# sarvex/redpanda

Hardware: AMD Instinct MI355X
Metric: record-batch validate+parse(+decompress) GB/s per GPU and per 8-GPU node (higher is better)
Workload: dtype u8; 1 GPU; C2: 1,048,576 uncompressed Kafka v2 batches x 16,381 B (16 records x (16 B key + 995 B value)), 4096 partitions per GPU; Kafka CRC32C + internal header CRC + record walk + offset/timestamp index; batches_per_gpu=1048576, batches_total=1048576, partitions_total=4096, partitions_per_gpu=4096, parallelism=partition-shard x1

## Files before the change

redpanda_amd/csrc/rpgpu_kernels.hip:

```cpp
#include "rpgpu_device.h"
#include "rpgpu_walk.h"

namespace rpgpu {

#ifdef RPGPU_DIAG_STAMPS
__device__ unsigned long long g_stamps[8];
struct Stamps {
    uint64_t st[8];
    uint64_t prev;
};
#define DIAG_PARAM , Stamps& sp
#define DIAG_PASS , sp
#define STAMP(i)                                          \
    do {                                                  \
        const uint64_t _t = __builtin_amdgcn_s_memtime(); \
        sp.st[i] += _t - sp.prev;                         \
        sp.prev = _t;                                     \
    } while (0)
#else
#define DIAG_PARAM
#define DIAG_PASS
#define STAMP(i) \
    do {         \
    } while (0)
#endif

struct Header {
    int32_t size_bytes;
    int64_t base_offset;
    int32_t type;
    int32_t crc;
    int16_t attrs;
    int32_t last_offset_delta;
    int64_t first_ts, max_ts, producer_id;
    int16_t producer_epoch;
    int32_t base_sequence, record_count;
};

struct Result {
    int32_t verdict;
    uint32_t crc, crc_expected, header_crc;
    Header h;
    uint32_t index_first, index_count;
};

__device__ __forceinline__ uint32_t u32s(uint32_t v) { return (uint32_t)__builtin_amdgcn_readfirstlane((int)v); }
__device__ __forceinline__ void write_result(rpgpu_batch_result* out, const Result& r) {
    if (lane_id() == 0) {
        const uint64_t bo = (uint64_t)r.h.base_offset, ft = (uint64_t)r.h.first_ts, mt = (uint64_t)r.h.max_ts;
        u32x4 a = {u32s((uint32_t)r.verdict), u32s(r.crc), u32s(r.crc_expected), u32s(r.header_crc)};
        u32x4 b = {u32s((uint32_t)r.h.size_bytes), u32s((uint32_t)r.h.record_count), u32s((uint32_t)bo),
                   u32s((uint32_t)(bo >> 32))};
        u32x4 c = {u32s((uint32_t)r.h.last_offset_delta),
                   u32s((uint32_t)(uint16_t)r.h.attrs | ((uint32_t)(r.h.attrs & 7) << 16) |
                        ((uint32_t)(uint8_t)r.h.type << 24)),
                   u32s((uint32_t)ft), u32s((uint32_t)(ft >> 32))};
        u32x4 d = {u32s((uint32_t)mt), u32s((uint32_t)(mt >> 32)), u32s(r.index_first), u32s(r.index_count)};
        u32x4* o = reinterpret_cast<u32x4*>(out);
        o[0] = a;
        o[1] = b;
        o[2] = c;
        o[3] = d;
    }
}

__device__ __forceinline__ void load_tables(uint32_t* s, const uint32_t* __restrict__ g) {
    for (int i = threadIdx.x; i < kTableWords / 4; i += blockDim.x)
        reinterpret_cast<u32x4*>(s)[i] = reinterpret_cast<const u32x4*>(g)[i];
    __syncthreads();
}

__device__ __forceinline__ uint32_t header_crc_vec(const uint32_t* sT, const Img64& D) {
    uint32_t win[16];
    win[0] = 0;
    win[1] = (D.w[1] << 24) ^ 0xff000000u;
    win[2] = ((D.w[1] >> 8) | (D.w[2] << 24)) ^ 0x00ffffffu;
#pragma unroll
    for (int m = 3; m < 16; m++) win[m] = (D.w[m - 1] >> 8) | (D.w[m] << 24);
    const uint32_t l = lane_id();
    uint32_t vwin = 0;
#pragma unroll
    for (int i = 0; i < 16; i++) vwin = writelane(vwin, win[i], i);
    const uint32_t w = __builtin_amdgcn_ds_bpermute((int)((l >> 2) << 2), vwin);
    const uint32_t byte = (w >> (8 * (l & 3))) & 255u;
    const uint32_t* hb = sT + kOffHB + l;
    uint32_t c = hb[(byte & 15u) * 64] ^ hb[(16u + (byte >> 4)) * 64];
    c ^= row_shl<1>(c);
    c ^= row_shl<2>(c);
    c ^= row_shl<4>(c);
    c ^= row_shl<8>(c);
    return ~(rdl(c, 0) ^ rdl(c, 16) ^ rdl(c, 32) ^ rdl(c, 48));
}

struct Geom {
    int32_t niter, g0;
};
__device__ __forceinline__ Geom geometry(int32_t n) {
    const int32_t niter = (n - 21 + 1023) >> 10;
    return Geom{niter, n - (niter << 10)};
}
__device__ __forceinline__ int32_t chunk_rows(int32_t niter) {
    return (niter + kRowsPerChunk - 1) & ~(kRowsPerChunk - 1);
}

struct Prefetch {
    u32x4 x[kRowsPerChunk];
    uint32_t hv;
    Geom gm;
};

typedef int32_t i32x4 __attribute__((ext_vector_type(4)));
__device__ __forceinline__ __amdgpu_buffer_rsrc_t batch_rsrc(const uint8_t* p) {
    return __builtin_amdgcn_make_buffer_rsrc(const_cast<uint8_t*>(p), 0, 0x7ffffff0, 0x00020000);
}
#ifndef RPGPU_ROW_AUX
#define RPGPU_ROW_AUX 2
#endif
__device__ __forceinline__ u32x4 load_row(__amdgpu_buffer_rsrc_t rs, const Geom& gm, int32_t row, uint32_t l) {
    const int32_t rb = row < gm.niter ? gm.g0 + (row << 10) : (int32_t)0x80000000;
    const i32x4 v = __builtin_amdgcn_raw_buffer_load_b128(rs, rb + (int32_t)(16 * l), 0, RPGPU_ROW_AUX);
    return (u32x4){(uint32_t)v.x, (uint32_t)v.y, (uint32_t)v.z, (uint32_t)v.w};
}

__device__ __forceinline__ void load_rows(u32x4 (&x)[kRowsPerChunk], __amdgpu_buffer_rsrc_t rs, const Geom& gm,
                                          int32_t cb, uint32_t l) {
#pragma unroll
    for (int k = 0; k < kRowsPerChunk; k++) x[k] = load_row(rs, gm, cb + k, l);
}

__device__ __forceinline__ Geom desc_geometry(const rpgpu_batch_desc& d) {
    return (d.length >= (uint32_t)kHeaderSize && !(d.flags & RPGPU_DESC_NULL_RECORDS)) ? geometry((int32_t)d.length)
                                                                                      : Geom{0, 0};
}

__device__ __forceinline__ u32x4 merge_header(u32x4 y, int32_t ro0, uint32_t v_img, uint32_t l) {
    if (ro0 >= kHeaderSize) return y;
    const int32_t ro = ro0 + 16 * (int32_t)l;
#pragma unroll
    for (int q = 0; q < 4; q++) {
        const int32_t o4 = ro + 4 * q;
        const uint32_t im = img_dword(v_img, o4);
        uint32_t keep;
        if (o4 >= kHeaderSize)
            keep = 0xffffffffu;
        else if (o4 + 4 <= kHeaderSize)
            keep = 0;
        else
            keep = 0xffffffffu << (8 * (uint32_t)(kHeaderSize - o4));
        const uint32_t raw = q == 0 ? y.x : q == 1 ? y.y : q == 2 ? y.z : y.w;
        const uint32_t v = (raw & keep) | (o4 >= kHeaderSize ? 0u : im);
        if (q == 0) y.x = v;
        if (q == 1) y.y = v;
        if (q == 2) y.z = v;
        if (q == 3) y.w = v;
    }
    return y;
}

__device__ __forceinline__ void process_batch(const uint32_t* __restrict__ sT, const rpgpu_batch_desc& d,
                                              uint32_t b, const uint8_t* __restrict__ data,
                                              rpgpu_batch_result* __restrict__ res, uint32_t index_first,
                                              Prefetch& pf, const rpgpu_batch_desc& nd,
                                              bool has_next DIAG_PARAM) {
    const uint32_t l = lane_id();
    const uint8_t* p = data + d.offset;
    const uint32_t len = d.length;
    Result r;
    r.verdict = RPGPU_V_OK;
    r.crc = r.crc_expected = r.header_crc = 0;
    r.h.size_bytes = r.h.type = r.h.crc = r.h.last_offset_delta = 0;
    r.h.base_sequence = r.h.record_count = 0;
    r.h.attrs = r.h.producer_epoch = 0;
    r.h.base_offset = r.h.first_ts = r.h.max_ts = r.h.producer_id = 0;
    r.index_first = index_first;
    r.index_count = 0;

    const uint32_t hv = pf.hv;
    Img64 H;
#pragma unroll
    for (int i = 0; i < 16; i++) H.w[i] = rdl(hv, i);
    Geom ngm{0, 0};
    const __amdgpu_buffer_rsrc_t nrs = batch_rsrc(data + (has_next ? nd.offset : 0));
    pf.hv = (uint32_t)__builtin_amdgcn_raw_buffer_load_b32(nrs, (int32_t)(4 * (l & 15)), 0, 0);
    if (has_next) ngm = desc_geometry(nd);

    Img64 D;
    D.clear();
    int64_t n;
    bool body_trunc = false;
    bool fail = false;
    if (d.flags & RPGPU_DESC_NULL_RECORDS) {
        n = 0;
        r.verdict = RPGPU_V_NULL_RECORDS;
        fail = true;
    } else if (d.format == RPGPU_FMT_KAFKA_WIRE) {
        const int32_t bl = (int32_t)H.get_be(8, 4);
        const uint64_t blen = (uint64_t)(int64_t)bl + 12u;
        if (blen <= (uint64_t)len) {
            n = (int64_t)blen;
        } else {
            n = len;
            body_trunc = true;
        }
        if (len < 12) {
            r.verdict = RPGPU_V_TOO_SMALL;
            fail = true;
        } else if (n < 17) {
            r.verdict = RPGPU_V_HDR_TRUNC_THROW;
            fail = true;
        } else if ((int8_t)H.byte(16) != 2) {
            r.verdict = RPGPU_V_BAD_MAGIC;
            fail = true;
        } else if (n < kHeaderSize) {
            r.verdict = RPGPU_V_HDR_TRUNC_THROW;
            fail = true;
        } else {
            r.h.size_bytes = (int32_t)((uint32_t)bl + 12u);
            r.h.base_offset = (int64_t)H.get_be(0, 8);
            r.h.type = 1;
            r.h.crc = (int32_t)H.get_be(17, 4);
            r.h.attrs = (int16_t)H.get_be(21, 2);
            r.h.last_offset_delta = (int32_t)H.get_be(23, 4);
            r.h.first_ts = (int64_t)H.get_be(27, 8);
            r.h.max_ts = (int64_t)H.get_be(35, 8);
            r.h.producer_id = (int64_t)H.get_be(43, 8);
            r.h.producer_epoch = (int16_t)H.get_be(51, 2);
            r.h.base_sequence = (int32_t)H.get_be(53, 4);
            r.h.record_count = (int32_t)H.get_be(57, 4);
            D.put_le(4, (uint32_t)r.h.size_bytes, 4);
            D.put_le(8, (uint64_t)r.h.base_offset, 8);
            D.put_le(16, 1, 1);
            D.put_le(17, (uint32_t)r.h.crc, 4);
            D.put_le(21, (uint16_t)r.h.attrs, 2);
            D.put_le(23, (uint32_t)r.h.last_offset_delta, 4);
            D.put_le(27, (uint64_t)r.h.first_ts, 8);
            D.put_le(35, (uint64_t)r.h.max_ts, 8);
            D.put_le(43, (uint64_t)r.h.producer_id, 8);
            D.put_le(51, (uint16_t)r.h.producer_epoch, 2);
            D.put_le(53, (uint32_t)r.h.base_sequence, 4);
            D.put_le(57, (uint32_t)r.h.record_count, 4);
        }
    } else {
        n = 0;
        if (len < kHeaderSize) {
            r.verdict = RPGPU_V_STREAM_SHORT;
            fail = true;
        } else {
            uint32_t any = 0;
#pragma unroll
            for (int i = 0; i < 15; i++) any |= H.w[i];
            any |= H.w[15] & 0xffu;
            if (any == 0) {
                r.verdict = RPGPU_V_FALLOCATED_ZERO;
                fail = true;
            } else {
#pragma unroll
                for (int i = 0; i < 16; i++) D.w[i] = H.w[i];
                D.w[15] &= 0xffu;
                r.h.size_bytes = (int32_t)H.get_le(4, 4);
                r.h.base_offset = (int64_t)H.get_le(8, 8);
                r.h.type = (int8_t)H.byte(16);
                r.h.crc = (int32_t)H.get_le(17, 4);
                r.h.attrs = (int16_t)H.get_le(21, 2);
                r.h.last_offset_delta = (int32_t)H.get_le(23, 4);
                r.h.first_ts = (int64_t)H.get_le(27, 8);
                r.h.max_ts = (int64_t)H.get_le(35, 8);
                r.h.producer_id = (int64_t)H.get_le(43, 8);
                r.h.producer_epoch = (int16_t)H.get_le(51, 2);
                r.h.base_sequence = (int32_t)H.get_le(53, 4);
                r.h.record_count = (int32_t)H.get_le(57, 4);
                n = (int64_t)r.h.size_bytes;
            }
        }
    }
    const bool is_disk = d.format != RPGPU_FMT_KAFKA_WIRE;
    const bool recrc = is_disk && (d.ops & RPGPU_OP_RECRC);
    if (!fail) {
        r.crc_expected = (uint32_t)r.h.crc;
        if (!recrc && ((d.ops & RPGPU_OP_HDRCRC) || is_disk)) r.header_crc = header_crc_vec(sT, D);
        if (is_disk) {
            if (!recrc && r.header_crc != H.w[0]) {
                r.verdict = RPGPU_V_HDR_CRC_MISMATCH;
                fail = true;
            } else if (r.h.size_bytes < kHeaderSize || (int64_t)r.h.size_bytes > (int64_t)len) {
                r.verdict = RPGPU_V_STREAM_SHORT;
                fail = true;
            }
        }
    }
    if (fail) {
        load_rows(pf.x, nrs, ngm, 0, l);
        pf.gm = ngm;
        write_result(res + b, r);
        return;
    }

    Img64 B;
    B.clear();
    B.put_be(21, (uint16_t)r.h.attrs, 2);
    B.put_be(23, (uint32_t)r.h.last_offset_delta, 4);
    B.put_be(27, (uint64_t)r.h.first_ts, 8);
    B.put_be(35, (uint64_t)r.h.max_ts, 8);
    B.put_be(43, (uint64_t)r.h.producer_id, 8);
    B.put_be(51, (uint16_t)r.h.producer_epoch, 2);
    B.put_be(53, (uint32_t)r.h.base_sequence, 4);
    B.put_be(57, (uint32_t)r.h.record_count, 4);
    B.w[5] ^= 0xffffff00u;
    B.w[6] ^= 0x000000ffu;
    uint32_t v_img = 0;
#pragma unroll
    for (int i = 0; i < 16; i++) v_img = (l == (uint32_t)i) ? B.w[i] : v_img;

    const Geom gm = geometry((int32_t)n);
    const int32_t nrows = chunk_rows(gm.niter);
    const bool pf_ok = pf.gm.niter == gm.niter && pf.gm.g0 == gm.g0;
    const uint32_t* sN = sT + kOffN;
    const __amdgpu_buffer_rsrc_t rs = batch_rsrc(p);
    const __amdgpu_buffer_rsrc_t nrs_rows = batch_rsrc(data + (has_next ? nd.offset : 0));
    uint32_t c = 0;
    STAMP(0);
    if (!pf_ok) load_rows(pf.x, rs, gm, 0, l);
    pf.x[0] = merge_header(pf.x[0], gm.g0, v_img, l);
    pf.x[1] = merge_header(pf.x[1], gm.g0 + 1024, v_img, l);
    for (int32_t cb = 0; cb < nrows; cb += kRowsPerChunk) {
        const bool last_chunk = cb + kRowsPerChunk >= nrows;
        const __amdgpu_buffer_rsrc_t lrs = last_chunk ? nrs_rows : rs;
        const Geom lg = last_chunk ? ngm : gm;
        const int32_t lrow = last_chunk ? 0 : cb + kRowsPerChunk;
#pragma unroll
        for (int k = 0; k < kRowsPerChunk; k++) {
            u32x4 y = pf.x[k];
            y.x ^= c;
            c = crc_block(sN, y);
            pf.x[k] = load_row(lrs, lg, lrow + k, l);
        }
    }
    pf.gm = ngm;
    STAMP(1);
#ifndef RPGPU_DIAG_NO_COMBINE
    c = combine64(sT + kOffW, c);
    if (nrows != gm.niter) c = apply8(sT + kOffU + (nrows - gm.niter) * 128, c);
#endif
    r.crc = ~rdl(c, 0);
#if defined(RPGPU_DIAG_NO_COMBINE) || defined(RPGPU_DIAG_NO_LOOKUP)
    asm volatile("" ::"v"(c));
    r.crc = r.crc_expected;
#endif
    if (recrc) {
        r.crc_expected = r.crc;
        r.h.crc = (int32_t)r.crc;
        D.put_le(17, r.crc, 4);
        r.header_crc = header_crc_vec(sT, D);
    }
    STAMP(2);

    const uint8_t codec = (uint8_t)(r.h.attrs & 7);
    if (r.crc != r.crc_expected) {
        r.verdict = RPGPU_V_CRC_MISMATCH;
    } else if (body_trunc) {
        r.verdict = RPGPU_V_BODY_TRUNC_THROW;
    } else if (codec > 4) {
        r.verdict = RPGPU_V_BAD_CODEC_THROW;
    }
    write_result(res + b, r);
    STAMP(3);
}

__global__ __launch_bounds__(kValidateThreads) void validate_kernel(
    const rpgpu_batch_desc* __restrict__ descs, uint32_t b0, uint32_t n, const uint8_t* __restrict__ data,
    rpgpu_batch_result* __restrict__ res, rpgpu_record_index* __restrict__ index,
    const uint32_t* __restrict__ local_first, const uint32_t* __restrict__ caps,
    const uint64_t* __restrict__ block_base, uint64_t index_cap, const uint32_t* __restrict__ tables) {
    __shared__ __attribute__((aligned(16))) uint32_t sT[kTableWords];
    load_tables(sT, tables);
    const uint32_t wave = threadIdx.x >> 6;
    const uint32_t gw = __builtin_amdgcn_readfirstlane(blockIdx.x * kWavesPerBlock + wave);
    const uint32_t nw = gridDim.x * kWavesPerBlock;
#ifdef RPGPU_DIAG_STAMPS
    Stamps sp{};
    sp.prev = __builtin_amdgcn_s_memtime();
#endif
    Prefetch pf;
    pf.gm = Geom{0, 0};
    if (b0 + gw < n) {
        const rpgpu_batch_desc d0 = sload_desc(descs + b0 + gw);
        const uint8_t* p0 = data + d0.offset;
        const __amdgpu_buffer_rsrc_t rs0 = batch_rsrc(p0);
        pf.hv = (uint32_t)__builtin_amdgcn_raw_buffer_load_b32(rs0, (int32_t)(4 * (lane_id() & 15)), 0, 0);
        pf.gm = desc_geometry(d0);
        load_rows(pf.x, rs0, pf.gm, 0, lane_id());
    }
    for (uint32_t b = b0 + gw; b < n; b += nw) {
        const rpgpu_batch_desc d = sload_desc(descs + b);
        const bool has_next = b + nw < n;
        const rpgpu_batch_desc nd = sload_desc(descs + (has_next ? b + nw : b));
        process_batch(sT, d, b, data, res, 0u, pf, nd, has_next DIAG_PASS);
        STAMP(5);
    }
#ifdef RPGPU_DIAG_STAMPS
    if (lane_id() == 0)
        for (int i = 0; i < 6; i++) atomicAdd(&g_stamps[i], (unsigned long long)sp.st[i]);
#endif
}

__global__ __launch_bounds__(256) void walk_kernel(const rpgpu_batch_desc* __restrict__ descs, uint32_t b0,
                                                   uint32_t n,
                                                   const uint8_t* __restrict__ data,
                                                   rpgpu_batch_result* __restrict__ res,
                                                   rpgpu_record_index* __restrict__ index,
                                                   const uint32_t* __restrict__ local_first,
                                                   const uint32_t* __restrict__ caps,
                                                   const uint64_t* __restrict__ block_base, uint64_t index_cap,
                                                   uint32_t* __restrict__ wave_list, uint32_t* __restrict__ wave_count) {
    const uint32_t b = b0 + blockIdx.x * blockDim.x + threadIdx.x;
    WalkJob J;
    J.flags = 0;
    J.body = 0;
    J.base_offset = J.first_ts = 0;
    J.n = J.first = J.cap = J.b = 0;
    J.rc = 0;
    uint32_t first_all = 0;
    if (b < n) {
        const rpgpu_batch_desc d = descs[b];
        const rpgpu_batch_result& r = res[b];
        const uint64_t first = block_base[b / kScanBlock] + local_first[b];
        first_all = (uint32_t)first;
        if ((d.ops & (RPGPU_OP_PARSE | RPGPU_OP_INDEX)) && r.verdict == RPGPU_V_OK && r.codec == 0) {
            uint64_t cap = caps[b];
            if (first >= index_cap) cap = 0;
            else if (first + cap > index_cap) cap = index_cap - first;
            J.body = d.offset + kHeaderSize;
            J.base_offset = r.base_offset;
            J.first_ts = r.first_timestamp;
            J.n = (uint32_t)r.size_bytes - kHeaderSize;
            J.rc = r.record_count;
            J.first = (uint32_t)first;
            J.cap = (uint32_t)cap;
            J.b = b;
            J.flags = kJobLive | ((d.ops & RPGPU_OP_INDEX) ? kJobIndex : 0u);
            if (J.rc > kWaveWalkMin) {
                wave_list[atomicAdd(wave_count, 1u)] = b;
                J.flags = 0;
            }
        }
    }
    walk_lanes(data, J, index, res);
    if (b < n && !(J.flags & kJobLive)) reinterpret_cast<uint32_t*>(res + b)[14] = first_all;
}

__global__ __launch_bounds__(256) void walk_wave_kernel(const rpgpu_batch_desc* __restrict__ descs,
                                                        const uint8_t* __restrict__ data,
                                                        rpgpu_batch_result* __restrict__ res,
                                                        rpgpu_record_index* __restrict__ index,
                                                        const uint32_t* __restrict__ local_first,
                                                        const uint32_t* __restrict__ caps,
                                                        const uint64_t* __restrict__ block_base, uint64_t index_cap,
                                                        const uint32_t* __restrict__ wave_list,
                                                        const uint32_t* __restrict__ wave_count,
                                                        uint32_t* __restrict__ head) {
    const uint32_t cnt = *wave_count;
    for (;;) {
        uint32_t k = 0;
        if (lane_id() == 0) k = atomicAdd(head, 1u);
        k = __builtin_amdgcn_readfirstlane(k);
        if (k >= cnt) break;
        const uint32_t b = wave_list[k];
        const rpgpu_batch_desc d = descs[b];
        const rpgpu_batch_result& r = res[b];
        const uint64_t first = block_base[b / kScanBlock] + local_first[b];
        uint64_t cap = caps[b];
        if (first >= index_cap) cap = 0;
        else if (first + cap > index_cap) cap = index_cap - first;
        WalkJob J;
        J.body = d.offset + kHeaderSize;
        J.base_offset = r.base_offset;
        J.first_ts = r.first_timestamp;
        J.n = (uint32_t)r.size_bytes - kHeaderSize;
        J.rc = r.record_count;
        J.first = (uint32_t)first;
        J.cap = (uint32_t)cap;
        J.b = b;
        J.flags = kJobLive | ((d.ops & RPGPU_OP_INDEX) ? kJobIndex : 0u);
        int32_t verdict;
        uint32_t count;
        wave_walk_batch(data, J, index, verdict, count);
        if (lane_id() == 0) {
            uint32_t* o = reinterpret_cast<uint32_t*>(res + b);
            o[0] = (uint32_t)verdict;
            o[15] = count;
        }
    }
}

__device__ __forceinline__ uint32_t index_cap(const rpgpu_batch_desc& d, const uint8_t* data) {
    if (!(d.ops & (RPGPU_OP_PARSE | RPGPU_OP_INDEX)) || (d.flags & RPGPU_DESC_NULL_RECORDS)) return 0;
    const uint8_t* p = data + d.offset;
    const uint64_t len = d.length;
    if (len < (uint64_t)kHeaderSize) return 0;
    uint64_t n;
    int32_t rc;
    uint32_t attrs;
    if (d.format == RPGPU_FMT_KAFKA_WIRE) {
        const int32_t bl = (int32_t)bswap32(ld4(p + 8));
        const uint64_t blen = (uint64_t)(int64_t)bl + 12u;
        if (blen > len) return 0;
        n = blen;
        if (n < (uint64_t)kHeaderSize || p[16] != 2) return 0;
        attrs = ((uint32_t)p[21] << 8) | p[22];
        rc = (int32_t)bswap32(ld4(p + 57));
    } else {
        const int32_t sz = (int32_t)ld4(p + 4);
        if (sz < kHeaderSize || (uint64_t)sz > len) return 0;
        n = (uint64_t)sz;
        attrs = ((uint32_t)p[22] << 8) | p[21];
        rc = (int32_t)ld4(p + 57);
    }
    if ((attrs & 7u) != 0 || rc <= 0) return 0;
    uint64_t cap = (n - kHeaderSize) / 2;
    if ((uint64_t)rc < cap) cap = (uint64_t)rc;
    return (uint32_t)cap;
}

__global__ __launch_bounds__(kScanBlock) void caps_kernel(const rpgpu_batch_desc* __restrict__ descs,
                                                          uint32_t n, const uint8_t* __restrict__ data,
                                                          uint32_t* __restrict__ caps,
                                                          uint32_t* __restrict__ local_first,
                                                          uint64_t* __restrict__ block_sum) {
    __shared__ uint32_t wsum[kScanBlock / 64];
    const uint32_t i = blockIdx.x * kScanBlock + threadIdx.x;
    uint32_t cap = 0;
    if (i < n) cap = index_cap(descs[i], data);
    const uint32_t l = lane_id();
    uint32_t x = cap;
#pragma unroll
    for (int s = 1; s < 64; s <<= 1) {
        uint32_t t = __shfl_up(x, s, 64);
        if (l >= (uint32_t)s) x += t;
    }
    const uint32_t wv = threadIdx.x >> 6;
    if (l == 63) wsum[wv] = x;
    __syncthreads();
    uint32_t wbase = 0;
    for (uint32_t k = 0; k < wv; k++) wbase += wsum[k];
    if (i < n) {
        caps[i] = cap;
        local_first[i] = wbase + x - cap;
    }
    if (threadIdx.x == kScanBlock - 1) {
        uint64_t tot = 0;
        for (uint32_t k = 0; k < kScanBlock / 64; k++) tot += wsum[k];
        block_sum[blockIdx.x] = tot;
    }
}

__global__ __launch_bounds__(1024) void block_scan_kernel(uint64_t* __restrict__ block_sum, uint32_t nb,
                                                          uint64_t* __restrict__ total_out) {
    __shared__ uint64_t part[1024];
    const uint32_t t = threadIdx.x;
    const uint32_t per = (nb + 1023) / 1024;
    const uint32_t lo = t * per, hi = (lo + per < nb) ? lo + per : nb;
    uint64_t s = 0;
    for (uint32_t k = lo; k < hi; k++) s += block_sum[k];
    part[t] = s;
    __syncthreads();
    for (uint32_t off = 1; off < 1024; off <<= 1) {
        uint64_t v = (t >= off) ? part[t - off] : 0;
        __syncthreads();
        part[t] += v;
        __syncthreads();
    }
    uint64_t run = part[t] - s;
    for (uint32_t k = lo; k < hi; k++) {
        const uint64_t v = block_sum[k];
        block_sum[k] = run;
        run += v;
    }
    if (t == 1023 && total_out) *total_out = part[1023];
}

__global__ __launch_bounds__(kValidateThreads) void crc_ranges_kernel(
    const uint8_t* __restrict__ data, const uint64_t* __restrict__ offs, const uint32_t* __restrict__ lens,
    const uint32_t* __restrict__ seeds, uint32_t n, uint32_t* __restrict__ out,
    const uint32_t* __restrict__ tables) {
    __shared__ __attribute__((aligned(16))) uint32_t sT[kTableWords];
    load_tables(sT, tables);
    const uint32_t l = lane_id();
    const uint32_t wave = threadIdx.x >> 6;
    const uint32_t gw = __builtin_amdgcn_readfirstlane(blockIdx.x * kWavesPerBlock + wave);
    const uint32_t nw = gridDim.x * kWavesPerBlock;
    for (uint32_t i = gw; i < n; i += nw) {
        const uint8_t* base = data + offs[i];
        const int64_t len = lens[i];
        const uint32_t init = ~(seeds ? seeds[i] : 0u);
        const uint32_t crc = crc_range_wave(sT, base, len, init, l);
        if (l == 0) out[i] = crc;
    }
}

__device__ __forceinline__ bool header_all_zero(const Img64& H) {
    uint32_t any = 0;
#pragma unroll
    for (int i = 0; i < 15; i++) any |= H.w[i];
    any |= H.w[15] & 0xffu;
    return any == 0;
}

__global__ __launch_bounds__(kValidateThreads) void segment_parse_kernel(
    const uint8_t* __restrict__ data, const rpgpu_segment_read* __restrict__ reads, uint32_t nreads,
    rpgpu_segment_parse_result* __restrict__ results, rpgpu_batch_desc* __restrict__ descs,
    const uint32_t* __restrict__ tables) {
    __shared__ __attribute__((aligned(16))) uint32_t sT[kTableWords];
    load_tables(sT, tables);
    const uint32_t l = lane_id();
    const uint32_t gw = __builtin_amdgcn_readfirstlane(blockIdx.x * kWavesPerBlock + (threadIdx.x >> 6));
    const uint32_t nw = gridDim.x * kWavesPerBlock;
    for (uint32_t s = gw; s < nreads; s += nw) {
        const rpgpu_segment_read rd = reads[s];
        const uint8_t* seg = data + rd.offset;
        const uint64_t len = rd.length;
        const bool reader = rd.mode == RPGPU_PARSE_READER;
        const uint64_t max_buffer = rd.max_buffer ? rd.max_buffer : 32u * 1024u;
        uint64_t pos = 0, bytes_consumed = 0, phys = 0, buffer = 0;
        int32_t err = RPGPU_V_OK;
        bool exception = false, stopped = false, over_budget = false;
        bool codec_throw = false;
        uint32_t accepted = 0, skipped = 0;
        int64_t start_offset = rd.start_offset, expected = rd.expected_next_batch;
        uint64_t cfg_bytes = rd.bytes_consumed;
        const __amdgpu_buffer_rsrc_t rs = batch_rsrc(seg);
        for (;;) {
            const uint64_t rem = len - pos;
            if (rem == 0) {
                err = RPGPU_V_END_OF_STREAM;
                break;
            }
            if (rem < (uint64_t)kHeaderSize) {
                err = RPGPU_V_STREAM_SHORT;
                break;
            }
            const uint32_t hv = (uint32_t)__builtin_amdgcn_raw_buffer_load_b32(rs, (int32_t)(pos + 4 * (l & 15)), 0, 0);
            Img64 H;
#pragma unroll
            for (int i = 0; i < 16; i++) H.w[i] = rdl(hv, i);
            if (header_all_zero(H)) {
                err = RPGPU_V_FALLOCATED_ZERO;
                break;
            }
            Img64 D;
#pragma unroll
            for (int i = 0; i < 16; i++) D.w[i] = H.w[i];
            D.w[15] &= 0xffu;
            if (header_crc_vec(sT, D) != H.w[0]) {
                err = RPGPU_V_HDR_CRC_MISMATCH;
                break;
            }
            const int32_t size_bytes = (int32_t)H.get_le(4, 4);
            const int64_t base_offset = (int64_t)H.get_le(8, 8);
            const int8_t type = (int8_t)H.byte(16);
            const int32_t lod = (int32_t)H.get_le(23, 4);
            const int64_t max_ts = (int64_t)H.get_le(35, 8);
            const int64_t last = base_offset + lod;
            const uint64_t sz = (uint64_t)(int64_t)size_bytes;
            int decision = 0;
            if (reader) {
                if (base_offset < expected) {
                    exception = true;
                    break;
                }
                if (base_offset > rd.max_offset) {
                    decision = 2;
                } else if ((rd.strict_max_bytes || cfg_bytes) && cfg_bytes + sz > rd.max_bytes) {
                    over_budget = true;
                    decision = 2;
                } else if (last < start_offset) {
                    decision = 1;
                } else if (rd.has_type_filter && rd.type_filter != type) {
                    start_offset = last + 1;
                    decision = 1;
                } else if (rd.has_first_timestamp && rd.first_timestamp > max_ts) {
                    start_offset = last + 1;
                    decision = 1;
                }
            }
            if (decision == 2) {
                stopped = true;
                break;
            }
            const uint64_t body = (uint64_t)((int64_t)size_bytes - kHeaderSize);
            const uint64_t avail = len - pos - kHeaderSize;
            if (decision == 1) {
                expected = last + 1;
                phys += sz;
                if (body > avail) {
                    err = RPGPU_V_STREAM_SHORT;
                    break;
                }
                pos += kHeaderSize + body;
                bytes_consumed += sz;
                skipped++;
                continue;
            }
            if (reader) expected = last + 1;
            phys += sz;
            const bool throws = reader && (H.byte(21) & 7u) > 4u && body <= avail;
            if (!throws && accepted < rd.desc_cap && l == 0) {
                rpgpu_batch_desc d;
                d.offset = rd.offset + pos;
                d.length = (uint32_t)(body > avail ? avail + kHeaderSize : body + kHeaderSize);
                d.partition = rd.partition;
                d.format = RPGPU_FMT_RP_DISK;
                d.ops = rd.ops;
                d.flags = 0;
                d.reserved = 0;
                descs[rd.desc_first + accepted] = d;
            }
            if (!throws) accepted++;
            bytes_consumed += sz;
            if (body > avail) {
                err = RPGPU_V_STREAM_SHORT;
                break;
            }
            pos += kHeaderSize + body;
            if (throws) {
                codec_throw = true;
                break;
            }
            if (reader) {
                start_offset = last + 1;
                cfg_bytes += sz;
                buffer += sz;
                if (last >= rd.stable_offset || last >= rd.max_offset ||
                    (rd.has_next_cached && rd.next_cached_batch == last + 1) || cfg_bytes >= rd.max_bytes ||
                    buffer >= max_buffer) {
                    stopped = true;
                    break;
                }
            }
        }
        if (l == 0) {
            rpgpu_segment_parse_result r;
            r.last_error = (exception || codec_throw) ? RPGPU_V_OK : err;
            const bool benign = err == RPGPU_V_OK || err == RPGPU_V_END_OF_STREAM || err == RPGPU_V_FALLOCATED_ZERO;
            r.status = exception     ? RPGPU_V_READ_OFFSET_REGRESSION
                       : codec_throw ? RPGPU_V_BAD_CODEC_THROW
                                     : ((bytes_consumed || benign) ? RPGPU_V_OK : err);
            r.accepted = accepted < rd.desc_cap ? accepted : rd.desc_cap;
            r.skipped = skipped;
            r.bytes_consumed = bytes_consumed;
            r.physical_offset = phys;
            r.start_offset = start_offset;
            r.cfg_bytes_consumed = cfg_bytes;
            r.expected_next_batch = expected;
            r.over_budget = over_budget;
            r.stopped = stopped;
            r.reserved0 = 0;
            r.reserved1 = 0;
            results[s] = r;
        }
    }
}

constexpr uint64_t kMaxConsumeSize = 128u * 1024u;
constexpr int8_t kTypeRaftData = 1, kTypeRaftConfiguration = 2, kTypeArchivalMetadata = 19;

__global__ __launch_bounds__(kValidateThreads) void remote_parse_kernel(
    const uint8_t* __restrict__ data, const rpgpu_remote_read* __restrict__ reads, uint32_t nreads,
    rpgpu_remote_parse_result* __restrict__ results, rpgpu_batch_desc* __restrict__ descs,
    int64_t* __restrict__ kafka_base, int64_t* __restrict__ gaps, const uint32_t* __restrict__ tables) {
    __shared__ __attribute__((aligned(16))) uint32_t sT[kTableWords];
    load_tables(sT, tables);
    const uint32_t l = lane_id();
    const uint32_t gw = __builtin_amdgcn_readfirstlane(blockIdx.x * kWavesPerBlock + (threadIdx.x >> 6));
    const uint32_t nw = gridDim.x * kWavesPerBlock;
    for (uint32_t s = gw; s < nreads; s += nw) {
        const rpgpu_remote_read rd = reads[s];
        const uint8_t* seg = data + rd.offset;
        const uint64_t len = rd.length;
        uint64_t pos = 0, bytes_consumed = 0, produced = 0;
        int32_t err = RPGPU_V_OK, thrown = RPGPU_V_OK;
        bool stopped = false, over_budget = rd.over_budget != 0;
        uint32_t accepted = 0, skipped = 0, ngaps = 0;
        int64_t start_offset = rd.start_offset, delta = rd.cur_delta, cur_rp = rd.cur_rp_offset;
        uint64_t cfg_bytes = rd.bytes_consumed;
        const __amdgpu_buffer_rsrc_t rs = batch_rsrc(seg);
        for (;;) {
            const uint64_t rem = len - pos;
            if (rem == 0) {
                err = RPGPU_V_END_OF_STREAM;
                break;
            }
            if (rem < (uint64_t)kHeaderSize) {
                err = RPGPU_V_STREAM_SHORT;
                break;
            }
            const uint32_t hv = (uint32_t)__builtin_amdgcn_raw_buffer_load_b32(rs, (int32_t)(pos + 4 * (l & 15)), 0, 0);
            Img64 H;
#pragma unroll
            for (int i = 0; i < 16; i++) H.w[i] = rdl(hv, i);
            if (header_all_zero(H)) {
                err = RPGPU_V_FALLOCATED_ZERO;
                break;
            }
            Img64 D;
#pragma unroll
            for (int i = 0; i < 16; i++) D.w[i] = H.w[i];
            D.w[15] &= 0xffu;
            if (header_crc_vec(sT, D) != H.w[0]) {
                err = RPGPU_V_HDR_CRC_MISMATCH;
                break;
            }
            const int32_t size_bytes = (int32_t)H.get_le(4, 4);
            const int64_t base_offset = (int64_t)H.get_le(8, 8);
            const int8_t type = (int8_t)H.byte(16);
            const uint32_t codec = H.byte(21) & 7u;
            const int32_t lod = (int32_t)H.get_le(23, 4);
            const int64_t max_ts = (int64_t)H.get_le(35, 8);
            const int64_t last = base_offset + lod;
            const uint64_t sz = (uint64_t)(int64_t)size_bytes;
            int decision = 0;
            if (base_offset < delta) {
                thrown = RPGPU_V_REMOTE_DELTA_ASSERT;
                break;
            }
            if (base_offset - delta > rd.max_offset) {
                decision = 2;
            } else if (type != kTypeRaftData) {
                decision = 1;
            } else if (last < delta) {
                thrown = RPGPU_V_REMOTE_DELTA_ASSERT;
                break;
            } else if (last - delta < start_offset) {
                decision = 1;
            } else if ((rd.strict_max_bytes || cfg_bytes) && cfg_bytes + sz > rd.max_bytes) {
                over_budget = true;
                decision = 2;
            } else if (rd.has_first_timestamp && rd.first_timestamp > max_ts) {
                decision = 1;
            }
            if (decision == 2) {
                stopped = true;
                break;
            }
            const uint64_t body = (uint64_t)((int64_t)size_bytes - kHeaderSize);
            const uint64_t avail = len - pos - kHeaderSize;
            if (decision == 1) {
                cur_rp = last + 1;
                if (type == kTypeRaftData && last - delta + 1 > start_offset) start_offset = last - delta + 1;
                if (type == kTypeRaftConfiguration || type == kTypeArchivalMetadata) {
                    if (ngaps < rd.gap_cap && l == 0) {
                        gaps[2 * ((uint64_t)rd.gap_first + ngaps)] = base_offset;
                        gaps[2 * ((uint64_t)rd.gap_first + ngaps) + 1] = last;
                    }
                    ngaps++;
                    delta += (int64_t)lod + 1;
                }
                if (body > avail) {
                    err = RPGPU_V_STREAM_SHORT;
                    break;
                }
                pos += kHeaderSize + body;
                bytes_consumed += sz;
                skipped++;
                continue;
            }
            bytes_consumed += sz;
            if (body > avail) {
                err = RPGPU_V_STREAM_SHORT;
                break;
            }
            const uint64_t bpos = pos;
            pos += kHeaderSize + body;
            if (codec > 4u) {
                thrown = RPGPU_V_BAD_CODEC_THROW;
                break;
            }
            cfg_bytes += sz;
            cur_rp = last + 1;
            if (last - delta + 1 > start_offset) start_offset = last - delta + 1;
            if (accepted < rd.desc_cap && l == 0) {
                rpgpu_batch_desc d;
                d.offset = rd.offset + bpos;
                d.length = (uint32_t)(body + kHeaderSize);
                d.partition = rd.partition;
                d.format = RPGPU_FMT_RP_DISK;
                d.ops = rd.ops;
                d.flags = 0;
                d.reserved = 0;
                descs[rd.desc_first + accepted] = d;
                kafka_base[rd.desc_first + accepted] = base_offset - delta;
            }
            accepted++;
            produced += sz;
            if (over_budget || produced > kMaxConsumeSize) {
                stopped = true;
                break;
            }
        }
        if (l == 0) {
            rpgpu_remote_parse_result r;
            const bool benign = err == RPGPU_V_OK || err == RPGPU_V_END_OF_STREAM || err == RPGPU_V_FALLOCATED_ZERO;
            r.last_error = thrown != RPGPU_V_OK ? RPGPU_V_OK : err;
            r.status = thrown != RPGPU_V_OK ? thrown : ((bytes_consumed || benign) ? RPGPU_V_OK : err);
            r.accepted = accepted < rd.desc_cap ? accepted : rd.desc_cap;
            r.skipped = skipped;
            r.bytes_consumed = bytes_consumed;
            r.start_offset = start_offset;
            r.cfg_bytes_consumed = cfg_bytes;
            r.cur_delta = delta;
            r.cur_rp_offset = cur_rp;
            r.produced_bytes = produced;
            r.gaps = ngaps;
            r.over_budget = over_budget;
            r.stopped = stopped;
            r.reserved = 0;
            results[s] = r;
        }
    }
}

hipError_t launch_remote_parse(const uint8_t* d_data, const rpgpu_remote_read* d_reads, uint32_t n,
                               rpgpu_remote_parse_result* d_res, rpgpu_batch_desc* d_descs, int64_t* d_kafka_base,
                               int64_t* d_gaps, const uint32_t* d_tables, int grid, hipStream_t s) {
    if (n == 0) return hipSuccess;
    const uint32_t need = (n + kWavesPerBlock - 1) / kWavesPerBlock;
    const uint32_t g = (uint32_t)grid < need ? (uint32_t)grid : need;
    remote_parse_kernel<<<g, kValidateThreads, 0, s>>>(d_data, d_reads, n, d_res, d_descs, d_kafka_base, d_gaps,
                                                       d_tables);
    return hipGetLastError();
}

hipError_t launch_segment_parse(const uint8_t* d_data, const rpgpu_segment_read* d_reads, uint32_t n,
                                rpgpu_segment_parse_result* d_res, rpgpu_batch_desc* d_descs,
                                const uint32_t* d_tables, int grid, hipStream_t s) {
    if (n == 0) return hipSuccess;
    const uint32_t need = (n + kWavesPerBlock - 1) / kWavesPerBlock;
    const uint32_t g = (uint32_t)grid < need ? (uint32_t)grid : need;
    segment_parse_kernel<<<g, kValidateThreads, 0, s>>>(d_data, d_reads, n, d_res, d_descs, d_tables);
    return hipGetLastError();
}

__global__ __launch_bounds__(256) void kafka_codes_kernel(const rpgpu_batch_result* __restrict__ res, uint32_t n,
                                                          uint32_t batch_max_bytes, int32_t* __restrict__ codes) {
    const uint32_t i = blockIdx.x * blockDim.x + threadIdx.x;
    if (i < n) codes[i] = kafka_error_code(res[i].verdict, res[i].size_bytes, batch_max_bytes);
}

hipError_t launch_kafka_codes(const rpgpu_batch_result* d_res, uint32_t n, uint32_t batch_max_bytes,
                              int32_t* d_codes, hipStream_t s) {
    if (n == 0) return hipSuccess;
    kafka_codes_kernel<<<(n + 255) / 256, 256, 0, s>>>(d_res, n, batch_max_bytes, d_codes);
    return hipGetLastError();
}

struct WaveWalk {
    uint32_t *list, *count;
};
static void scratch_parts(void* d_scratch, uint32_t n, uint32_t** caps, uint32_t** local_first,
                          uint64_t** block_sum, WaveWalk* ww = nullptr) {
    uint8_t* sc = static_cast<uint8_t*>(d_scratch);
    *caps = reinterpret_cast<uint32_t*>(sc);
    *local_first = *caps + n;
    const size_t o_bs = ((size_t)n * 8 + 15) & ~(size_t)15;
    *block_sum = reinterpret_cast<uint64_t*>(sc + o_bs);
    const size_t nb = (n + kScanBlock - 1) / kScanBlock;
    const size_t o_ww = (o_bs + nb * 8 + 63) & ~(size_t)63;
    if (ww) {
        ww->count = reinterpret_cast<uint32_t*>(sc + o_ww);
        ww->list = ww->count + 16;
    }
}

hipError_t launch_plan(const rpgpu_batch_desc* d_descs, uint32_t n, const uint8_t* d_data,
                       uint64_t* d_index_used, void* d_scratch, hipStream_t s) {
    if (n == 0) {
        if (d_index_used) return hipMemsetAsync(d_index_used, 0, sizeof(uint64_t), s);
        return hipSuccess;
    }
    const uint32_t nb = (n + kScanBlock - 1) / kScanBlock;
    uint32_t *caps, *local_first;
    uint64_t* block_sum;
    scratch_parts(d_scratch, n, &caps, &local_first, &block_sum);
    caps_kernel<<<nb, kScanBlock, 0, s>>>(d_descs, n, d_data, caps, local_first, block_sum);
    block_scan_kernel<<<1, 1024, 0, s>>>(block_sum, nb, d_index_used);
    return hipGetLastError();
}

hipError_t launch_block_scan(uint64_t* block_sum, uint32_t nb, uint64_t* total, hipStream_t s) {
    block_scan_kernel<<<1, 1024, 0, s>>>(block_sum, nb, total);
    return hipGetLastError();
}

hipError_t launch_run(const rpgpu_batch_desc* d_descs, uint32_t n, const uint8_t* d_data,
                      rpgpu_batch_result* d_res, rpgpu_record_index* d_index, uint64_t index_cap,
                      const void* d_scratch, const uint32_t* d_tables, int grid, hipStream_t s,
                      const Overlap* ov) {
    if (n == 0) return hipSuccess;
    uint32_t *caps, *local_first;
    uint64_t* block_sum;
    WaveWalk ww;
    scratch_parts(const_cast<void*>(d_scratch), n, &caps, &local_first, &block_sum, &ww);
    hipError_t e = hipSuccess;
    const uint32_t chunks = (ov && n >= kRunChunkMin) ? (uint32_t)ov->chunks : 1u;
    if ((e = hipMemsetAsync(ww.count, 0, 2 * sizeof(uint32_t), s)) != hipSuccess) return e;
    hipStream_t ws = s;
    for (uint32_t k = 0; k < chunks; k++) {
        const uint32_t lo = (uint32_t)((uint64_t)n * k / chunks), hi = (uint32_t)((uint64_t)n * (k + 1) / chunks);
        const uint32_t need = (hi - lo + kWavesPerBlock - 1) / kWavesPerBlock;
        const uint32_t g = (uint32_t)grid < need ? (uint32_t)grid : need;
        validate_kernel<<<g, kValidateThreads, 0, s>>>(d_descs, lo, hi, d_data, d_res, d_index, local_first, caps,
                                                        block_sum, index_cap, d_tables);
        if ((e = hipGetLastError()) != hipSuccess) return e;
        if (chunks > 1) {
            if ((e = hipEventRecord(ov->ev[k], s)) != hipSuccess) return e;
            if ((e = hipStreamWaitEvent(ov->aux, ov->ev[k], 0)) != hipSuccess) return e;
            ws = ov->aux;
        }
        walk_kernel<<<(hi - lo + 255) / 256, 256, 0, ws>>>(d_descs, lo, hi, d_data, d_res, d_index, local_first,
                                                           caps, block_sum, index_cap, ww.list, ww.count);
        if ((e = hipGetLastError()) != hipSuccess) return e;
    }
    {
        const uint32_t wg = (n < 1024u ? (n + 3) / 4 : 256u);
        walk_wave_kernel<<<wg, 256, 0, ws>>>(d_descs, d_data, d_res, d_index, local_first, caps, block_sum, index_cap,
                                             ww.list, ww.count, ww.count + 1);
        if ((e = hipGetLastError()) != hipSuccess) return e;
    }
    if (chunks > 1) {
        if ((e = hipEventRecord(ov->ev[chunks], ov->aux)) != hipSuccess) return e;
        if ((e = hipStreamWaitEvent(s, ov->ev[chunks], 0)) != hipSuccess) return e;
    }
    return hipSuccess;
}

hipError_t launch_validate(const rpgpu_batch_desc* d_descs, uint32_t n, const uint8_t* d_data,
                           rpgpu_batch_result* d_res, rpgpu_record_index* d_index, uint64_t index_cap,
                           uint64_t* d_index_used, void* d_scratch, const uint32_t* d_tables, int grid,
                           hipStream_t s, const Overlap* ov) {
    hipError_t e;
    if (ov && n >= kRunChunkMin) {
        if ((e = hipEventRecord(ov->ev[ov->chunks], s)) != hipSuccess) return e;
        if ((e = hipStreamWaitEvent(ov->aux, ov->ev[ov->chunks], 0)) != hipSuccess) return e;
        if ((e = launch_plan(d_descs, n, d_data, d_index_used, d_scratch, ov->aux)) != hipSuccess) return e;
    } else if ((e = launch_plan(d_descs, n, d_data, d_index_used, d_scratch, s)) != hipSuccess) {
        return e;
    }
    return launch_run(d_descs, n, d_data, d_res, d_index, index_cap, d_scratch, d_tables, grid, s, ov);
}

hipError_t launch_crc_ranges(const uint8_t* d_data, const uint64_t* d_off, const uint32_t* d_len,
                             const uint32_t* d_seed, uint32_t n, uint32_t* d_out, const uint32_t* d_tables,
                             int grid, hipStream_t s) {
    if (n == 0) return hipSuccess;
    const uint32_t need = (n + kWavesPerBlock - 1) / kWavesPerBlock;
    const uint32_t g = (uint32_t)grid < need ? (uint32_t)grid : need;
    crc_ranges_kernel<<<g, kValidateThreads, 0, s>>>(d_data, d_off, d_len, d_seed, n, d_out, d_tables);
    return hipGetLastError();
}

hipError_t validate_occupancy(int* blocks_per_cu) {
    return hipOccupancyMaxActiveBlocksPerMultiprocessor(blocks_per_cu, validate_kernel, kValidateThreads, 0);
}

size_t validate_scratch_bytes(uint32_t n) {
    const size_t nb = (n + kScanBlock - 1) / kScanBlock;
    return (((((size_t)n * 8 + 15) & ~(size_t)15) + nb * 8 + 63) & ~(size_t)63) + 64 + (size_t)n * 4 + 64;
}

}

#ifdef RPGPU_DIAG_STAMPS
extern "C" int rpgpu_diag_stamps(unsigned long long* out) {
    unsigned long long z[8] = {};
    if (hipMemcpyFromSymbol(out, HIP_SYMBOL(rpgpu::g_stamps), sizeof(z)) != hipSuccess) return -1;
    return hipMemcpyToSymbol(HIP_SYMBOL(rpgpu::g_stamps), z, sizeof(z)) == hipSuccess ? 0 : -1;
}
#endif
```

Measured before the change: 3990 GB/s.

## Skip header image build for wire batches and pipeline descriptor loads

For non-disk (wire) batches, the per-lane header image built with big-endian puts and a 16-way select is no longer constructed. The first rows are instead masked with a cheap mask_wire so the Kafka CRC covers only bytes from offset 21 onward, with the 0xffffffff init folded in. The validate loop also rotates batch descriptors through registers and loads the descriptor two iterations ahead, so scalar descriptor latency stays off the critical path. Waves with no work now exit early, and correctness depends on mask_wire reproducing the CRC seeding the old merge_header path did.

After: 4049 GB/s, median of 6. Within noise of the previous version (+1.5%).

```diff
diff --git a/redpanda_amd/csrc/rpgpu_kernels.hip b/redpanda_amd/csrc/rpgpu_kernels.hip
--- a/redpanda_amd/csrc/rpgpu_kernels.hip
+++ b/redpanda_amd/csrc/rpgpu_kernels.hip
@@ -149,6 +149,27 @@
             keep = 0xffffffffu << (8 * (uint32_t)(kHeaderSize - o4));
         const uint32_t raw = q == 0 ? y.x : q == 1 ? y.y : q == 2 ? y.z : y.w;
         const uint32_t v = (raw & keep) | (o4 >= kHeaderSize ? 0u : im);
+        if (q == 0) y.x = v;
+        if (q == 1) y.y = v;
+        if (q == 2) y.z = v;
+        if (q == 3) y.w = v;
+    }
+    return y;
+}
+
+__device__ __forceinline__ uint32_t bytes_from(int32_t o4, int32_t x) {
+    return o4 >= x ? 0xffffffffu : (o4 + 4 <= x ? 0u : 0xffffffffu << (8 * (uint32_t)(x - o4)));
+}
+__device__ __forceinline__ u32x4 mask_wire(u32x4 y, int32_t ro0, uint32_t l) {
+    if (ro0 >= 25) return y;
+    const int32_t ro = ro0 + 16 * (int32_t)l;
+#pragma unroll
+    for (int q = 0; q < 4; q++) {
+        const int32_t o4 = ro + 4 * q;
+        const uint32_t keep = bytes_from(o4, 21);
+        const uint32_t init = keep & ~bytes_from(o4, 25);
+        const uint32_t raw = q == 0 ? y.x : q == 1 ? y.y : q == 2 ? y.z : y.w;
+        const uint32_t v = (raw & keep) ^ init;
         if (q == 0) y.x = v;
         if (q == 1) y.y = v;
         if (q == 2) y.z = v;
@@ -295,21 +316,23 @@
         return;
     }
 
-    Img64 B;
-    B.clear();
-    B.put_be(21, (uint16_t)r.h.attrs, 2);
-    B.put_be(23, (uint32_t)r.h.last_offset_delta, 4);
-    B.put_be(27, (uint64_t)r.h.first_ts, 8);
-    B.put_be(35, (uint64_t)r.h.max_ts, 8);
-    B.put_be(43, (uint64_t)r.h.producer_id, 8);
-    B.put_be(51, (uint16_t)r.h.producer_epoch, 2);
-    B.put_be(53, (uint32_t)r.h.base_sequence, 4);
-    B.put_be(57, (uint32_t)r.h.record_count, 4);
-    B.w[5] ^= 0xffffff00u;
-    B.w[6] ^= 0x000000ffu;
     uint32_t v_img = 0;
-#pragma unroll
-    for (int i = 0; i < 16; i++) v_img = (l == (uint32_t)i) ? B.w[i] : v_img;
+    if (is_disk) {
+        Img64 B;
+        B.clear();
+        B.put_be(21, (uint16_t)r.h.attrs, 2);
+        B.put_be(23, (uint32_t)r.h.last_offset_delta, 4);
+        B.put_be(27, (uint64_t)r.h.first_ts, 8);
+        B.put_be(35, (uint64_t)r.h.max_ts, 8);
+        B.put_be(43, (uint64_t)r.h.producer_id, 8);
+        B.put_be(51, (uint16_t)r.h.producer_epoch, 2);
+        B.put_be(53, (uint32_t)r.h.base_sequence, 4);
+        B.put_be(57, (uint32_t)r.h.record_count, 4);
+        B.w[5] ^= 0xffffff00u;
+        B.w[6] ^= 0x000000ffu;
+#pragma unroll
+        for (int i = 0; i < 16; i++) v_img = (l == (uint32_t)i) ? B.w[i] : v_img;
+    }
 
     const Geom gm = geometry((int32_t)n);
     const int32_t nrows = chunk_rows(gm.niter);
@@ -320,8 +343,13 @@
     uint32_t c = 0;
     STAMP(0);
     if (!pf_ok) load_rows(pf.x, rs, gm, 0, l);
-    pf.x[0] = merge_header(pf.x[0], gm.g0, v_img, l);
-    pf.x[1] = merge_header(pf.x[1], gm.g0 + 1024, v_img, l);
+    if (is_disk) {
+        pf.x[0] = merge_header(pf.x[0], gm.g0, v_img, l);
+        pf.x[1] = merge_header(pf.x[1], gm.g0 + 1024, v_img, l);
+    } else {
+        pf.x[0] = mask_wire(pf.x[0], gm.g0, l);
+        pf.x[1] = mask_wire(pf.x[1], gm.g0 + 1024, l);
+    }
     for (int32_t cb = 0; cb < nrows; cb += kRowsPerChunk) {
         const bool last_chunk = cb + kRowsPerChunk >= nrows;
         const __amdgpu_buffer_rsrc_t lrs = last_chunk ? nrs_rows : rs;
@@ -380,21 +408,22 @@
     Stamps sp{};
     sp.prev = __builtin_amdgcn_s_memtime();
 #endif
+    if (b0 + gw >= n) return;
+    rpgpu_batch_desc d = sload_desc(descs + b0 + gw);
+    rpgpu_batch_desc nd = sload_desc(descs + (b0 + gw + nw < n ? b0 + gw + nw : b0 + gw));
     Prefetch pf;
-    pf.gm = Geom{0, 0};
-    if (b0 + gw < n) {
-        const rpgpu_batch_desc d0 = sload_desc(descs + b0 + gw);
-        const uint8_t* p0 = data + d0.offset;
-        const __amdgpu_buffer_rsrc_t rs0 = batch_rsrc(p0);
+    {
+        const __amdgpu_buffer_rsrc_t rs0 = batch_rsrc(data + d.offset);
         pf.hv = (uint32_t)__builtin_amdgcn_raw_buffer_load_b32(rs0, (int32_t)(4 * (lane_id() & 15)), 0, 0);
-        pf.gm = desc_geometry(d0);
+        pf.gm = desc_geometry(d);
         load_rows(pf.x, rs0, pf.gm, 0, lane_id());
     }
     for (uint32_t b = b0 + gw; b < n; b += nw) {
-        const rpgpu_batch_desc d = sload_desc(descs + b);
         const bool has_next = b + nw < n;
-        const rpgpu_batch_desc nd = sload_desc(descs + (has_next ? b + nw : b));
+        const rpgpu_batch_desc nnd = sload_desc(descs + (b + 2 * nw < n ? b + 2 * nw : b));
         process_batch(sT, d, b, data, res, 0u, pf, nd, has_next DIAG_PASS);
+        d = nd;
+        nd = nnd;
         STAMP(5);
     }
 #ifdef RPGPU_DIAG_STAMPS
```
